# Mictronics/pluto-gps-sim

Hardware: AMD Instinct MI355X
Metric: IQ samples/sec (whole node) at 16 channels; bit-exact int16 IQ vs CPU ref (higher is better)
Workload: dtype f64 NCOs (exact), i32 accumulate of packed int16 I/Q

## Files before the change

### pluto-gps-sim_amd/csrc/gpsbb.hip

```cpp
#include <hip/hip_runtime.h>

#include <algorithm>
#include <cctype>
#include <cmath>
#include <cstdio>
#include <cstdlib>
#include <cstring>
#include <new>
#include <condition_variable>
#include <functional>
#include <mutex>
#include <thread>
#include <chrono>
#include <vector>

#include "gpsbb.h"
#include "gpsbb_kernels.hip.h"
#include "gpsbb_noise.hip.h"
#include "gpsbb_interf.hip.h"
#include "gpsbb_level.hip.h"
#include "gpsbb_events.hip.h"
#include "gpsbb_dense.hip.h"
#include "gpsbb_despread.hip.h"
#include "gpsbb_walk.hip.h"
// ... 9 lines not shown
#ifdef GPSBB_EXPERIMENTS
#define GPSBB_KNOB_LONG(name, dflt) ([](long d) -> long { static const char *const e = getenv(name); return e ? atol(e) : d; }((long)(dflt)))
#define GPSBB_KNOB_SET(name) ([]() -> bool { static const bool v = getenv(name) != nullptr; return v; }())
#else
#define GPSBB_KNOB_LONG(name, dflt) ((long)(dflt))
#define GPSBB_KNOB_SET(name) (false)
#endif


namespace {

constexpr uint64_t kSinCosFnv1a = 0x1c99a5cf84551314ull;

bool make_sincos(int32_t sin512[512], int32_t cos512[512])
{
    const double two_pi = 6.283185307179586476925286766559;
    for (int i = 0; i < 512; i++) {
        const double a = two_pi * (double)i / 512.0;
        sin512[i] = (int32_t)(511.0 * std::sin(a) + 1.0);
        cos512[i] = (int32_t)(511.0 * std::cos(a) + 1.0);
    }
    uint64_t h = 0xcbf29ce484222325ull;
    auto eat = [&h](const int32_t *t) {
        for (int i = 0; i < 512; i++)
            for (int k = 0; k < 4; k++) {
                h ^= (uint8_t)((uint32_t)t[i] >> (8 * k));
                h *= 0x100000001b3ull;
            }
    };
    eat(sin512);
    eat(cos512);
    return h == kSinCosFnv1a;
}

const uint8_t kG2Taps[32][2] = {
    {2, 6}, {3, 7}, {4, 8}, {5, 9}, {1, 9}, {2, 10}, {1, 8}, {2, 9}, {3, 10}, {2, 3}, {3, 4},
    {5, 6}, {6, 7}, {7, 8}, {8, 9}, {9, 10}, {1, 4}, {2, 5}, {3, 6}, {4, 7}, {5, 8}, {6, 9},
    {1, 3}, {4, 6}, {5, 7}, {6, 8}, {7, 9}, {8, 10}, {1, 6}, {2, 7}, {3, 8}, {4, 9}};

void make_ca(int prn, uint8_t ca[GPSBB_CA_LEN])
{
    uint32_t g1 = 0x3ff, g2 = 0x3ff;
    const int t1 = kG2Taps[prn - 1][0], t2 = kG2Taps[prn - 1][1];
    for (int i = 0; i < GPSBB_CA_LEN; i++) {
        const uint32_t o1 = (g1 >> 9) & 1u;
        const uint32_t o2 = ((g2 >> (t1 - 1)) ^ (g2 >> (t2 - 1))) & 1u;
        ca[i] = (uint8_t)(o1 ^ o2);
        const uint32_t f1 = ((g1 >> 2) ^ (g1 >> 9)) & 1u;
        const uint32_t f2 = ((g2 >> 1) ^ (g2 >> 2) ^ (g2 >> 5) ^ (g2 >> 7) ^ (g2 >> 8) ^ (g2 >> 9)) & 1u;
        g1 = ((g1 << 1) | f1) & 0x3ff;
        g2 = ((g2 << 1) | f2) & 0x3ff;
    }
}

bool chan_ok(const gpsbb_chan_t &c, double delt, bool fixed = false)
{
    if (c.prn == 0)
        return true;
    if (c.prn < 0 || c.prn > 32)
        return false;
    if (!std::isfinite(c.f_carr) || !std::isfinite(c.f_code) || !std::isfinite(c.carr_phase) ||
        !std::isfinite(c.code_phase) || !std::isfinite(c.gain))
        return false;
    if (!fixed && (std::signbit(c.carr_phase) || c.carr_phase > 1.0))
        return false;
    if (fixed && (std::signbit(c.carr_phase) || c.carr_phase >= 4294967296.0 || c.carr_phase != std::floor(c.carr_phase)))
        return false;
    if (std::signbit(c.code_phase) || !(c.code_phase < 1023.0))
        return false;
    const double sc = c.f_code * delt, sk = c.f_carr * delt;
    if (!(sc > 0.0 && sc <= 1.5) || !(std::fabs(sk) <= 0.125))
        return false;
    if (!(std::fabs(c.gain) < 2097152.0))
        return false;
    if (c.iword < 0 || c.iword > 59 || c.ibit < 0 || c.ibit > 29 || c.icode < 0 || c.icode > 19)
        return false;
    for (int k = 0; k < GPSBB_N_DWRD; k++)
        if (c.dwrd[k] >> 30)
            return false;
    return true;
}

uint64_t row_bound(double s_abs, double range, int top_e, int nsamp)
{
    if (!(s_abs > 0.0))
        return 4;
    int es;
    std::frexp(s_abs, &es);
    es -= 1;
    const double laps = std::floor((double)nsamp * s_abs / range) + 2.0;
    int binades = top_e - es + 3;
    if (binades < 3)
        binades = 3;
    const double per_lap = 2.0 * binades + 6.0;
    return (uint64_t)(laps * per_lap) + 16;
}

struct CarrDrift {
    int e_lo = 0, n = 0;
    double sa = 0.0, R1 = 0.0;
    bool neg = false;
    double dens[64], cum[65];
    explicit CarrDrift(double s)
    {
        sa = std::fabs(s);
        neg = s < 0.0;
        if (!(sa >= 0x1p-60) || !(sa < 0.25))
            return;
        int es;
        std::frexp(sa, &es);
        es -= 1;
        e_lo = es - 1 < -1 ? es - 1 : -1;
        cum[0] = 0.0;
        for (int e = e_lo; e <= -1; e++) {
            const double ulp = std::ldexp(1.0, e - 52);
            const double q = s / ulp;
            const double delta = (std::nearbyint(q) - q) * ulp;
            dens[n] = delta / sa;
            cum[n + 1] = cum[n] + dens[n] * std::ldexp(1.0, e);
            n++;
        }
        R1 = cum[n];
    }
    double R(double x) const
    {
        if (n == 0 || !(x > std::ldexp(1.0, e_lo)))
            return 0.0;
        if (x >= 1.0)
            return R1;
        const int e = std::ilogb(x);
        const int k = e - e_lo;
        return cum[k] + dens[k] * (x - std::ldexp(1.0, e));
    }
    double advance(double x0, int nsteps, double s) const
    {
        const double u = x0 + (double)nsteps * s;
        const double fl = std::floor(u), end = u - fl;
        const double drift = neg ? -fl * R1 + R(x0) - R(end) : fl * R1 + R(end) - R(x0);
        double v = end + drift;
        v -= std::floor(v);
        return v;
    }
};

double ev_bias_on_grid(double w)
{
#ifdef GPSBB_W_OFF_GRID
    return w;
#else
    return w < 0.25 ? std::ceil(w * 4294967296.0) * 0x1p-32 : w;
#endif
}

bool ev_plan(const gpsbb_chan_t *ch, int nblocks, int nch, double delt, std::vector<EvConst> &out, bool fixed = false)
{
    const size_t nbc = (size_t)nblocks * nch;
    out.resize(nbc);
    const double reach = (double)SPT - 0.5;
    for (int blk = 0; blk < nblocks; blk++) {
        double amp_sum = 0.0;
        for (int i = 0; i < nch; i++) {
            const gpsbb_chan_t &c = ch[(size_t)blk * nch + i];
            EvConst &K = out[(size_t)blk * nch + i];
            memset(&K, 0, sizeof K);
            if (c.prn <= 0)
                continue;
            amp_sum += 512.0 * std::fabs(c.gain) + 1.0;
            const volatile double sc = c.f_code * delt, sk = c.f_carr * delt;
            double S = sk * 512.0;
            if (fixed) {
                const volatile double scaled = 512.0 * 65536.0 * c.f_carr * delt;
                S = (double)(int)std::round(scaled) * 0x1p-16;
            }
            const double aS = std::fabs(S);
            const bool dense_code = !(sc * reach < 1.0);
            if (!(sc >= 0x1p-20) || !(1023.0 + 1040.0 * sc + 2.0 <= (double)EV_CHIP_LEN))
                return false;
            K.S = aS;
            K.sc = sc;
            K.rsc = 1.0 / sc;
            K.down = S < 0.0;
            const double wC = EV_MODEL_ERR * K.rsc + EV_T_EPS;
            double wK = 0.0;
            if (aS == 0.0) {
                K.rS = 0x1p+1000;
                K.kc = 1;
            } else if (aS < 8.0 * EV_MODEL_ERR) {
                K.rS = 0x1p+1000;
                K.kc = -1;
            } else {
                K.rS = 1.0 / aS;
                wK = EV_MODEL_ERR * K.rS + EV_T_EPS;
                const double kc = std::floor((reach + wK) * aS) + 1.0;
                K.kc = kc > (double)EV_KC_MAX ? EV_KC_DENSE : (int)kc;
            }
            K.W = std::max(std::max(wK, wC), EV_T_EPS);
            K.W = ev_bias_on_grid(K.W);
            K.danger = K.W >= 0.25 ? 0x80000000u : (uint32_t)std::ceil(2.0 * K.W * 4294967296.0) + 1u;
            {
                const long floor_ = GPSBB_KNOB_LONG("GPSBB_EV_DANGER", 0);
                if (floor_ > 0 && (uint32_t)floor_ > K.danger)
                    K.danger = (uint32_t)floor_;
            }
            K.tK0 = K.rS * (1.0 + K.W) + 0x1p+20 + K.W;
            K.tC0 = K.rsc * (1.0 + K.W) + 0x1p+20 + K.W;
            K.pd_S8 = aS * 8.0;
            K.pd_dy = aS * 512.0;
            K.pd_sc2 = sc * 2.0;
            K.pd_dx = sc * 128.0;
            if (dense_code && K.kc > 0)
                K.kc = EV_KC_DENSE;
            if (fixed) {
                if (dense_code) {
                    if (!(aS < 64.0))
                        return false;
                    K.kc = EV_KC_DENSE;
                } else {
                    const double kc = std::floor(reach * aS) + 1.0;
                    if (kc > (double)EV_KC_MAX)
                        return false;
                    K.kc = (int)kc;
                    K.rS = aS > 0.0 ? 1.0 / aS : 0x1p+1000;
                    K.W = ev_bias_on_grid(std::max(wC, EV_T_EPS));
                    K.danger = K.W >= 0.25 ? 0x80000000u : (uint32_t)std::ceil(2.0 * K.W * 4294967296.0) + 1u;
                    K.tK0 = K.rS * (1.0 - 0x1p-17) + 0x1p+20;
                    K.tC0 = K.rsc * (1.0 + K.W) + 0x1p+20 + K.W;
                }
            }
            K.danger_le = K.kc < 0 ? 0xffffffffu : K.danger - 1u;
            K.chip_at = (uint32_t)(offsetof(EvLdsLean, chip2) + (size_t)i * sizeof(uint16_t) * EvLdsLean::CHIPS) - (EV_GUARD_HI << 1);
            K.amp_at = (uint32_t)(offsetof(EvLdsLean, amp) + (size_t)i * sizeof(uint32_t) * EvLdsLean::AMP) - (EV_GUARD_HI << 2);
        }
        if (!(amp_sum < 32768.0))
            return false;
    }
    return true;
}

bool lap_eligible(const gpsbb_chan_t *ch, size_t nbc, double delt, bool fixed)
{
    for (size_t k = 0; k < nbc; k++) {
        const gpsbb_chan_t &c = ch[k];
        if (c.prn <= 0)
            continue;
        const volatile double sc = c.f_code * delt, sk = c.f_carr * delt;
        if (!(sc >= 0x1p-20))
            return false;
        if (!fixed && !(std::fabs(sk) >= 0x1p-50) && sk != 0.0)
            return false;
    }
    return true;
}

constexpr int LAP_UNIT_CARR = 4, LAP_UNIT_CODE = 2;
constexpr int LAP_BURST_SHARE = 4;
int lap_unit(int kind, size_t nbc)
{
    long u = kind == NCO_CARR ? GPSBB_KNOB_LONG("GPSBB_LAP_UNIT_CARR", LAP_UNIT_CARR) : GPSBB_KNOB_LONG("GPSBB_LAP_UNIT_CODE", LAP_UNIT_CODE);
    if (nbc <= 256)
        u = 1;
    else if (nbc <= 1024)
        u = kind == NCO_CARR ? std::min(u, 2L) : 1L;
    if (kind == NCO_CODE && u == 0)
        return 0;
    return u < 1 ? 1 : (u > 64 ? 64 : (int)u);
}

void lap_bound(const gpsbb_chan_t *ch, int nblocks, int nch, double delt, int nsamp, bool fixed, uint32_t chunk0[2][GPSBB_MAX_CHAN + 1],
               bool carr_only = false)
{
    for (int kind = 0; kind < 2; kind++) {
        chunk0[kind][0] = kind == 0 ? 0u : chunk0[0][GPSBB_MAX_CHAN];
        for (int i = 0; i < nch; i++) {
            double laps = 0.0;
            for (int blk = 0; blk < nblocks; blk++) {
                const gpsbb_chan_t &c = ch[(size_t)blk * nch + i];
                if (c.prn <= 0 || (kind == NCO_CARR && fixed) || (kind == NCO_CODE && carr_only))
                    continue;
                const double s = kind == NCO_CARR ? std::fabs(c.f_carr * delt) : c.f_code * delt * (1.0 / 1023.0);
                laps += std::floor((std::floor((double)nsamp * s * (1.0 + 0x1p-30)) + 1.0) / (double)std::max(1, lap_unit(kind, (size_t)nblocks * nch))) + 3.0;
            }
            const uint32_t chunks = (uint32_t)((laps + (double)(LAP_WG - 1)) / (double)LAP_WG) + 1u;
            chunk0[kind][i + 1] = chunk0[kind][i] + chunks;
        }
        for (int i = nch; i < GPSBB_MAX_CHAN; i++)
            chunk0[kind][i + 1] = chunk0[kind][i];
    }
}

}


struct WorkPool {
    std::vector<std::thread> th;
    std::mutex m;
    std::condition_variable cv_work, cv_done;
    std::function<void(size_t)> job;
    size_t njobs = 0, next = 0, running = 0;
    unsigned long gen = 0;
    bool stop = false;

    explicit WorkPool(size_t nworkers)
    {
        for (size_t t = 0; t < nworkers; t++)
            th.emplace_back([this] { loop(); });
    }
    ~WorkPool()
    {
        {
            std::lock_guard<std::mutex> g(m);
            stop = true;
        }
        cv_work.notify_all();
        for (auto &t : th)
            t.join();
    }
    void loop()
    {
        unsigned long seen = 0;
        std::unique_lock<std::mutex> lk(m);
        for (;;) {
            cv_work.wait(lk, [&] { return stop || gen != seen; });
            if (stop)
                return;
            seen = gen;
            drain(lk);
        }
    }
    void drain(std::unique_lock<std::mutex> &lk)
    {
        running++;
        while (next < njobs) {
            const size_t j = next++;
            lk.unlock();
            job(j);
            lk.lock();
        }
        if (--running == 0)
            cv_done.notify_all();
    }
    void run(size_t n, std::function<void(size_t)> f)
    {
        std::unique_lock<std::mutex> lk(m);
        job = std::move(f);
        njobs = n;
        next = 0;
        gen++;
// ... 391 lines not shown
        (void)hipFree(h->d_pack);
    if (h->d_noise_tab)
        (void)hipFree(h->d_noise_tab);
    if (h->d_nclip)
        (void)hipFree(h->d_nclip);
    if (h->d_digest.p)
        (void)hipFree(h->d_digest.p);
    if (h->d_level)
        (void)hipFree(h->d_level);
    delete h->pool;
    h->pool = nullptr;
    for_each_stream(h, [](hipStream_t st) { (void)hipStreamDestroy(st); });
    delete h;
}

static hipError_t create_seed_stream(hipStream_t *st);

#ifdef GPSBB_EXPERIMENTS
__global__ void k_park(unsigned long long ticks)
{
    const unsigned long long t0 = wall_clock64();
    while (wall_clock64() - t0 < ticks)
        __builtin_amdgcn_s_sleep(64);
}
#endif

static hipError_t zero_now(gpsbb *h, void *ptr, size_t bytes)
{
#ifdef GPSBB_EXPERIMENTS
    {
        const long park = GPSBB_KNOB_LONG("GPSBB_X_PARK_NULL_MS", 0);
        if (park > 0)
            hipLaunchKernelGGL(k_park, dim3(1), dim3(1), 0, nullptr, (unsigned long long)park * 100000ull);
        if (GPSBB_KNOB_SET("GPSBB_X_NULL_MEMSET"))
            return hipMemsetAsync(ptr, 0, bytes, nullptr);
    }
#endif
    const hipError_t e = hipMemsetAsync(ptr, 0, bytes, h->s_seed);
    return e != hipSuccess ? e : hipStreamSynchronize(h->s_seed);
}

typedef void (*EvKernelFn)(BatchDev, int16_t *);
static EvKernelFn ev_kernel(int g, bool digest);

extern "C" int gpsbb_create(gpsbb_t **out, int device)
{
    if (!out)
        return GPSBB_E_BADARG;
    *out = nullptr;
    int ndev = 0;
    if (hipGetDeviceCount(&ndev) != hipSuccess || ndev <= 0 || device < 0 || device >= ndev)
        return GPSBB_E_NODEVICE;

    int32_t tabs[1024];
    if (!make_sincos(tabs + 512, tabs))
        return GPSBB_E_INTERNAL;
    std::vector<uint32_t> ca(33 * 32, 0u);
    for (int prn = 1; prn <= 32; prn++) {
        uint8_t chips[GPSBB_CA_LEN];
        make_ca(prn, chips);
        for (int i = 0; i < GPSBB_CA_LEN; i++)
            if (chips[i])
                ca[prn * 32 + (i >> 5)] |= 1u << (i & 31);
    }

    gpsbb *h = new (std::nothrow) gpsbb;
    if (!h)
        return GPSBB_E_NOMEM;
    h->device = device;
    auto fail = [&](hipError_t e) {
        h->last_hip = (int)e;
        gpsbb_destroy(h);
        return e == hipErrorOutOfMemory ? GPSBB_E_NOMEM : GPSBB_E_HIP;
    };
    hipError_t e;
    if ((e = hipSetDevice(device)) != hipSuccess) return fail(e);
    hipDeviceProp_t prop;
    if ((e = hipGetDeviceProperties(&prop, device)) != hipSuccess) return fail(e);
    h->sm_count = prop.multiProcessorCount;
    if ((e = create_seed_stream(&h->s_seed)) != hipSuccess) return fail(e);
    {
        const long sp = GPSBB_KNOB_LONG("GPSBB_SYNTH_STREAM_PRIO", 0);
        if (sp != 0) {
            if ((e = hipStreamCreateWithPriority(&h->s_compute, hipStreamNonBlocking, (int)sp)) != hipSuccess) return fail(e);
        } else {
            if ((e = hipStreamCreateWithFlags(&h->s_compute, hipStreamNonBlocking)) != hipSuccess) return fail(e);
        }
    }
    if ((e = create_seed_stream(&h->s_more[0])) != hipSuccess) return fail(e);
    if ((e = hipMalloc((void **)&h->d_tabs, sizeof tabs)) != hipSuccess) return fail(e);
    if ((e = hipMalloc((void **)&h->d_ca, ca.size() * 4)) != hipSuccess) return fail(e);
    if ((e = hipMalloc((void **)&h->d_status, 4)) != hipSuccess) return fail(e);
    if ((e = hipMalloc((void **)&h->d_hz, 64)) != hipSuccess) return fail(e);
    if ((e = hipMalloc((void **)&h->d_clip, 8)) != hipSuccess) return fail(e);
    if ((e = hipMemcpy(h->d_tabs, tabs, sizeof tabs, hipMemcpyHostToDevice)) != hipSuccess) return fail(e);
    if ((e = hipMemcpy(h->d_ca, ca.data(), ca.size() * 4, hipMemcpyHostToDevice)) != hipSuccess) return fail(e);
    if ((e = hipStreamSynchronize(nullptr)) != hipSuccess) return fail(e);
    h->h_ca = ca;
    if ((e = zero_now(h, h->d_status, 4)) != hipSuccess) return fail(e);
    if ((e = zero_now(h, h->d_hz, 64)) != hipSuccess) return fail(e);
    if ((e = zero_now(h, h->d_clip, 8)) != hipSuccess) return fail(e);
    if ((e = hipFuncSetAttribute(reinterpret_cast<const void *>(k_synth), hipFuncAttributeMaxDynamicSharedMemorySize,
                                 (int)sizeof(SynthLds))) != hipSuccess) return fail(e);
    for (int g = 0; g <= EV_STATE_LOG2_MAX; g++) {
        if ((e = hipFuncSetAttribute(reinterpret_cast<const void *>(ev_kernel(g, false)), hipFuncAttributeMaxDynamicSharedMemorySize,
                                     (int)sizeof(EvLdsLean) + EV_PICK_LDS)) != hipSuccess) return fail(e);
        if ((e = hipFuncSetAttribute(reinterpret_cast<const void *>(ev_kernel(g, true)), hipFuncAttributeMaxDynamicSharedMemorySize,
                                     (int)sizeof(EvLdsLean) + EV_PICK_LDS)) != hipSuccess) return fail(e);
    }
    if ((e = hipFuncSetAttribute(reinterpret_cast<const void *>(k_synth_ev_dense), hipFuncAttributeMaxDynamicSharedMemorySize,
                                 (int)sizeof(EvLds) + EV_PICK_LDS)) != hipSuccess) return fail(e);
    if ((e = hipFuncSetAttribute(reinterpret_cast<const void *>(k_synth_ev_fixed), hipFuncAttributeMaxDynamicSharedMemorySize,
                                 (int)sizeof(EvLdsLean) + EV_PICK_LDS)) != hipSuccess) return fail(e);
    if ((e = hipFuncSetAttribute(reinterpret_cast<const void *>(k_synth_pd<true>), hipFuncAttributeMaxDynamicSharedMemorySize,
                                 (int)sizeof(PdLds<true>) + EV_PICK_LDS)) != hipSuccess) return fail(e);
    if ((e = hipFuncSetAttribute(reinterpret_cast<const void *>(k_synth_pd<false>), hipFuncAttributeMaxDynamicSharedMemorySize,
                                 (int)sizeof(PdLds<false>) + EV_PICK_LDS)) != hipSuccess) return fail(e);
    if ((e = hipFuncSetAttribute(reinterpret_cast<const void *>(k_synth_pd<true, true>), hipFuncAttributeMaxDynamicSharedMemorySize,
                                 (int)sizeof(PdLds<true>) + EV_PICK_LDS)) != hipSuccess) return fail(e);
    if ((e = hipFuncSetAttribute(reinterpret_cast<const void *>(k_synth_pd<false, true>), hipFuncAttributeMaxDynamicSharedMemorySize,
                                 (int)sizeof(PdLds<false>) + EV_PICK_LDS)) != hipSuccess) return fail(e);
    *out = h;
    return GPSBB_OK;
}

struct ChainCarry {
    int prn[GPSBB_MAX_CHAN];
    double phase[GPSBB_MAX_CHAN];
};
static void chain_carrier_host(const gpsbb_chan_t *ch, int nblocks, int nch, double delt, int nsamp, double *seed,
                               int nthreads, ChainCarry *carry);

static bool host_seeding_wanted(const gpsbb_batch *b);

typedef void (*LapKernelFn)(BatchDev, LapDev);
static LapKernelFn lap_pass2_kernel(int kind, bool wide, int g)
{
#define GPSBB_P2(W) {{k_lap_pass2<NCO_CODE, W, 0>, k_lap_pass2<NCO_CODE, W, 1>, k_lap_pass2<NCO_CODE, W, 2>}, \
                     {k_lap_pass2<NCO_CARR, W, 0>, k_lap_pass2<NCO_CARR, W, 1>, k_lap_pass2<NCO_CARR, W, 2>}, \
                     {k_lap_pass2_2<W, 0>, k_lap_pass2_2<W, 1>, k_lap_pass2_2<W, 2>}}
    static const LapKernelFn k[2][3][EV_STATE_LOG2_MAX + 1] = {GPSBB_P2(false), GPSBB_P2(true)};
#undef GPSBB_P2
    static_assert(NCO_CODE == 0 && NCO_CARR == 1, "lap_pass2_kernel's table");
    return k[wide ? 1 : 0][kind < 0 ? 2 : kind][g];
}

static EvKernelFn ev_kernel(int g, bool digest)
{
    static const EvKernelFn k[2][EV_STATE_LOG2_MAX + 1] = {{k_synth_ev<0>, k_synth_ev<1>, k_synth_ev<2>},
                                                            {k_synth_ev_digest<0>, k_synth_ev_digest<1>, k_synth_ev_digest<2>}};
    return k[digest ? 1 : 0][g];
}

static int ev_state_log2(const gpsbb_batch *b, bool fixed)
{
    if (!b->ev || !b->laps || b->ev_dense || fixed)
        return 0;
    long g = GPSBB_KNOB_LONG("GPSBB_EV_STATE_LOG2", GPSBB_EV_STATE_LOG2);
    g = g < 0 ? 0 : (g > EV_STATE_LOG2_MAX ? EV_STATE_LOG2_MAX : g);
    while (g > 0 && !ev_granule_fits((int)g))
        g--;
    const size_t nbc = (size_t)b->nblocks * b->nch;
    for (size_t k = 0; k < nbc && g > 0; k++)
        if (!(b->h_evc[k].sc * (double)((TILE << g) + SPT) < (double)(GPSBB_CA_LEN - 1)))
            return 0;
    return (int)g;
}

struct PushTrace {
    double limit_ms = -1.0;
    int n = 0;
    const char *what[32];
    std::chrono::steady_clock::time_point t[32];
    PushTrace()
    {
#ifdef GPSBB_EXPERIMENTS
        const char *e = getenv("GPSBB_PUSH_TRACE");
        if (e)
            limit_ms = atof(e);
#endif
    }
    void start() { n = 0; mark("start"); }
    void mark(const char *w)
    {
        if (limit_ms < 0.0 || n >= 32)
            return;
        what[n] = w;
        t[n++] = std::chrono::steady_clock::now();
    }
    void end()
    {
        if (limit_ms < 0.0 || n < 2)
            return;
        mark("end");
        const double tot = std::chrono::duration<double, std::milli>(t[n - 1] - t[0]).count();
        if (tot < limit_ms)
            return;
        fprintf(stderr, "[gpsbb push %.3f ms]", tot);
        for (int i = 1; i < n; i++)
            fprintf(stderr, " %s %.3f", what[i], std::chrono::duration<double, std::milli>(t[i] - t[i - 1]).count());
        fprintf(stderr, "\n");
    }
};
static thread_local PushTrace g_push_trace;
#define PUSH_MARK(w) g_push_trace.mark(w)

static hipError_t stage_upload(gpsbb_batch *b, void *dst, const void *src, size_t bytes, hipStream_t stream)
{
    const size_t at = (b->stage_used + 63) & ~(size_t)63;
    if (at + bytes > b->stage_cap)
        return hipMemcpyAsync(dst, src, bytes, hipMemcpyHostToDevice, stream);
    memcpy(b->stage + at, src, bytes);
    b->stage_used = at + bytes;
    return hipMemcpyAsync(dst, b->stage + at, bytes, hipMemcpyHostToDevice, stream);
}


static int batch_setup(gpsbb_batch *b, const gpsbb_chan_t *ch, int nblocks, int nch, double delt,
                       int nsamp, unsigned flags, hipStream_t upload_stream)
{
    gpsbb *h = b->h;
    if (!ch || nblocks < 1 || nblocks > 65535 || nch < 1 || nch > GPSBB_MAX_CHAN || nsamp < 1 ||
        !(delt > 0.0) || !std::isfinite(delt) || (flags & ~(GPSBB_CHAIN_CARRIER | GPSBB_FIXED_CARRIER)))
        return GPSBB_E_BADARG;
    const size_t nbc = (size_t)nblocks * nch;
    const bool fixed = (flags & GPSBB_FIXED_CARRIER) != 0;
    for (size_t k = 0; k < nbc; k++)
        if (!chan_ok(ch[k], delt, fixed))
            return GPSBB_E_BADCHAN;

    {
        const size_t need = nbc * (sizeof(gpsbb_chan_t) + sizeof(EvConst) + 8 + 2 * 4 + 5 * 4 +
                                   (size_t)CHAIN_SEG_MAX * (sizeof(ChainDesc) + 8 + 8 + 2 * 4)) + 64 * 1024;
        if (b->upload_done)
            HIPCHK(h, hipEventSynchronize(b->upload_done));
        PUSH_MARK("arena");
        if (need > b->stage_cap) {
            if (b->stage)
                (void)hipHostFree(b->stage);
            b->stage = nullptr;
            b->stage_cap = 0;
            HIPCHK(h, hipHostMalloc((void **)&b->stage, need + need / 4, hipHostMallocDefault));
            b->stage_cap = need + need / 4;
        }
        b->stage_used = 0;
    }
    b->nblocks = nblocks;
    b->nch = nch;
    b->nsamp = nsamp;
    b->delt = delt;
    b->flags = flags;
    b->ntiles = (nsamp + TILE - 1) / TILE;
    if (2ull * nbc * ((unsigned long long)b->ntiles + 1) >= (1ull << 32))
        return GPSBB_E_NOMEM;

    b->ev = h->opt_synth_kernel != 1 && ev_plan(ch, nblocks, nch, delt, b->h_evc, fixed);
    b->ev_dense = false;
    b->ev_all_dense = b->ev;
    if (b->ev)
        for (size_t k = 0; k < nbc; k++) {
            b->ev_dense = b->ev_dense || b->h_evc[k].kc == EV_KC_DENSE;
            b->ev_all_dense = b->ev_all_dense && (ch[k].prn <= 0 || b->h_evc[k].kc == EV_KC_DENSE);
        }
    b->ev_all_dense = b->ev_all_dense && b->ev_dense;
    if (fixed && b->ev_dense && !b->ev_all_dense) {
        b->ev = false;
        b->ev_dense = b->ev_all_dense = false;
    }
    PUSH_MARK("ev_plan");

    const bool lap_ok = b->ev && h->opt_seed_where != 1 && h->opt_seed_where != 2 && h->opt_chain_where != 2 && h->opt_chain_where != 3 &&
                        !GPSBB_KNOB_SET("GPSBB_NO_LAPS") && lap_eligible(ch, nbc, delt, fixed);
    b->host_seed = !lap_ok && !b->d_carry && host_seeding_wanted(b);
    b->laps = lap_ok;
    b->st_log2 = ev_state_log2(b, fixed);
    b->nstates = (b->ntiles + (1 << b->st_log2) - 1) >> b->st_log2;
    const bool chained = !fixed && (flags & GPSBB_CHAIN_CARRIER) && (nblocks > 1 || b->d_carry);
    b->chain_dev = chained && h->opt_chain_where != 1 && !b->host_seed;
    b->chain_fix_seq = h->opt_chain_where == 2;
    b->chain_starts = b->chain_dev && !b->ev;
    b->chain_model = false;
    b->chain_indep = false;
    b->nseg = 1;
    const bool indep_ok = !chained && !b->d_carry && b->ev && !fixed && !b->host_seed && h->opt_chain_where == 0 &&
                          b->ntiles >= (int)GPSBB_KNOB_LONG("GPSBB_INDEP_MIN_TILES", CHAIN_INDEP_MIN_TILES);
    if (!b->laps && ((b->chain_dev && !b->chain_starts) || indep_ok)) {
        double rows_max = 0.0;
        for (size_t k = 0; k < nbc; k++)
            if (ch[k].prn > 0) {
                const double sa = std::fabs(ch[k].f_carr * delt);
                const double r = sa > 0.0 ? ((double)nsamp * sa + 1.0) * (2.0 - std::log2(sa)) : 1.0;
                rows_max = r > rows_max ? r : rows_max;
            }
        int n = (int)(rows_max / (double)GPSBB_KNOB_LONG("GPSBB_SEG_ROWS", CHAIN_SEG_ROWS) + 0.5);
        const int n_cap = b->ntiles / CHAIN_SEG_MIN_TILES;
        n = n > CHAIN_SEG_MAX ? CHAIN_SEG_MAX : n;
        n = n > n_cap ? n_cap : n;
        n = n < 1 ? 1 : n;
        if (b->chain_dev) {
            b->nseg = n;
        } else if (n > 1 && (long)nblocks * n <= CHAIN_MODEL_MAX_SEGS) {
            b->chain_dev = true;
            b->chain_indep = true;
            b->nseg = n;
        }
    }
    b->seg_tiles = (b->ntiles + b->nseg - 1) / b->nseg;
    b->nseg = (b->ntiles + b->seg_tiles - 1) / b->seg_tiles;
    b->chain_model = !b->laps && b->chain_dev && !b->chain_starts && !b->d_carry && h->opt_chain_where != 3 &&
                     (long)nblocks * b->nseg <= CHAIN_MODEL_MAX_SEGS;
    const size_t nvbc = nbc * (size_t)b->nseg;

    b->row_off.assign(nbc + nvbc + 1, 0);
    uint64_t off = 0;
    for (size_t k = 0; k < nbc && !b->laps; k++) {
        b->row_off[k] = off;
        if (ch[k].prn > 0) {
            off += row_bound(ch[k].f_code * delt, 1023.0, 9, nsamp) + 1;
            if (b->ev)
                off += (uint64_t)nsamp / (uint64_t)WALK_ROW_MAX + 1;
        } else {
            off += 1;
        }
    }
    if (!b->laps) {
        const int full = b->seg_tiles * TILE, last = nsamp - (b->nseg - 1) * full;
        const int ns_full = b->nseg == 1 ? nsamp : full, ns_last = b->nseg == 1 ? nsamp : last;
        for (int blk = 0; blk < nblocks; blk++)
            for (int sgi = 0; sgi < b->nseg; sgi++) {
                uint64_t *ro = &b->row_off[nbc + ((size_t)blk * b->nseg + sgi) * nch];
                const int ns = sgi == b->nseg - 1 ? ns_last : ns_full;
                for (int i = 0; i < nch; i++) {
                    const gpsbb_chan_t &c = ch[(size_t)blk * nch + i];
                    ro[i] = 0;
                    if (c.prn > 0 && !fixed) {
                        if (sgi == 0 || sgi == b->nseg - 1)
                            ro[i] = row_bound(std::fabs(c.f_carr * delt), 1.0, -1, ns) + 1 + (b->ev ? (uint64_t)ns / (uint64_t)WALK_ROW_MAX + 1 : 0);
                        else
                            ro[i] = b->row_off[nbc + ((size_t)blk * b->nseg) * nch + i];
                    } else {
                        ro[i] = 1;
                    }
                }
            }
        for (size_t kv = 0; kv < nvbc; kv++) {
            const uint64_t cnt = b->row_off[nbc + kv];
            b->row_off[nbc + kv] = off;
            off += cnt;
        }
    }
    b->row_off[nbc + nvbc] = off;
    b->total_rows = off;

    HIPCHK(h, (hipError_t)b->d_ch.reserve(nbc));
    HIPCHK(h, (hipError_t)b->d_row_off.reserve(nbc + nvbc + 1));
    HIPCHK(h, (hipError_t)b->d_tile_ctr.reserve((size_t)NSETS * ((size_t)nblocks + 1)));
    b->nsets = (int)GPSBB_KNOB_LONG("GPSBB_NSETS", b->chain_dev ? 4 : 3);
    b->nsets = b->nsets < 2 ? 2 : (b->nsets > NSETS ? NSETS : b->nsets);
    b->nsets = b->nsets > b->max_sets ? b->max_sets : b->nsets;
    for (int set = 0; set < b->nsets; set++) {
        HIPCHK(h, (hipError_t)b->d_end[set].reserve(nbc));
        if (b->ev) {
            HIPCHK(h, (hipError_t)b->d_tile_x[set].reserve(2 * nbc * (size_t)b->nstates));
            HIPCHK(h, (hipError_t)b->d_tile_nav[set].reserve(nbc * (size_t)b->nstates));
            HIPCHK(h, (hipError_t)b->d_rows[set].reserve(b->total_rows + 4, b->max_sets == 1 ? (size_t)(b->total_rows / 2) : 0));
            HIPCHK(h, (hipError_t)b->d_row_cnt[set].reserve(nbc + nvbc));
        } else {
            HIPCHK(h, (hipError_t)b->d_rows[set].reserve(b->total_rows + 4));
            HIPCHK(h, (hipError_t)b->d_tile_row[set].reserve(2 * nbc * ((size_t)b->ntiles + 1)));
            HIPCHK(h, (hipError_t)b->d_row_cnt[set].reserve(2 * nbc));
        }
    }
    if (b->ev) {
        HIPCHK(h, (hipError_t)b->d_evc.reserve(nbc));
        HIPCHK(h, stage_upload(b, b->d_evc.p, b->h_evc.data(), nbc * sizeof(EvConst), upload_stream));
    }
    if (fixed) {
        b->h_kph0.assign(nbc, 0u);
        b->h_kstep.assign(nbc, 0);
        for (int i = 0; i < nch; i++) {
            int prev_prn = b->fixed_prev_prn ? b->fixed_prev_prn[i] : 0;
            uint32_t prev_ph = b->fixed_prev_phase ? b->fixed_prev_phase[i] : 0u;
            for (int blk = 0; blk < nblocks; blk++) {
                const gpsbb_chan_t &c = ch[(size_t)blk * nch + i];
                const size_t k = (size_t)blk * nch + i;
                if (c.prn <= 0) {
                    prev_prn = 0;
                    continue;
                }
                const volatile double scaled = 512.0 * 65536.0 * c.f_carr * delt;
                b->h_kstep[k] = (int)std::round(scaled);
                const bool cont = (flags & GPSBB_CHAIN_CARRIER) && c.prn == prev_prn;
                b->h_kph0[k] = cont ? prev_ph : (uint32_t)c.carr_phase;
                prev_ph = b->h_kph0[k] + (uint32_t)nsamp * (uint32_t)b->h_kstep[k];
                prev_prn = c.prn;
            }
        }
        HIPCHK(h, (hipError_t)b->d_kph0.reserve(nbc));
        HIPCHK(h, (hipError_t)b->d_kstep.reserve(nbc));
        HIPCHK(h, stage_upload(b, b->d_kph0.p, b->h_kph0.data(), nbc * 4, upload_stream));
        HIPCHK(h, stage_upload(b, b->d_kstep.p, b->h_kstep.data(), nbc * 4, upload_stream));
    }
    b->h_ch.assign(ch, ch + nbc);
    b->cont0_mask = 0;
    if (b->laps) {
        lap_bound(ch, nblocks, nch, delt, nsamp, fixed, b->lap_chunk0);
        const size_t chunks = (size_t)b->lap_chunk0[1][nch];
        for (int set = 0; set < b->nsets; set++) {
            HIPCHK(h, (hipError_t)b->d_lap_bc[set].reserve(2 * nbc));
            HIPCHK(h, (hipError_t)b->d_lap_lane0[set].reserve(2 * (size_t)nch * ((size_t)nblocks + 1)));
            HIPCHK(h, (hipError_t)b->d_lap_cnt[set].reserve(4 * GPSBB_MAX_CHAN));
            HIPCHK(h, (hipError_t)b->d_lap_rec[set].reserve(chunks * LAP_WG, b->max_sets == 1 ? chunks * LAP_WG / 4 : 0));
            HIPCHK(h, (hipError_t)b->d_lap_agg[set].reserve(chunks, b->max_sets == 1 ? chunks / 4 : 0));
            HIPCHK(h, (hipError_t)b->d_lap_chunk_m[set].reserve(chunks, b->max_sets == 1 ? chunks / 4 : 0));
            HIPCHK(h, (hipError_t)b->d_lap_chunk_bad[set].reserve(chunks, b->max_sets == 1 ? chunks / 4 : 0));
        }
        if (b->chain_dev && b->d_carry && b->carry_prn)
            for (int i = 0; i < nch; i++)
                if (ch[i].prn > 0 && ch[i].prn == b->carry_prn[i])
                    b->cont0_mask |= 1u << i;
    }
    if (b->chain_dev && !b->laps) {
        b->h_cd.resize(nvbc);
        b->h_start0.resize(nvbc);
        for (int i = 0; i < nch; i++) {
            double x = b->d_carry && b->carry_phase ? b->carry_phase[i] : 0.0;
            int prev_prn = b->d_carry && b->carry_prn ? b->carry_prn[i] : 0;
            for (int blk = 0; blk < nblocks; blk++) {
// ... 2955 lines not shown
};
}

extern "C" int gpsbb_test_build_rows(int kind, double x0, double s, unsigned nav0, int nsamp,
                                     gpsbb_test_row_t *rows, int cap, double *x_end, unsigned *nav_end)
{
    HostSink sink{rows, cap, 0, 0};
    uint32_t nav = nav0;
    double x = kind == NCO_CODE ? build_rows<NCO_CODE>(x0, s, nav, nsamp, sink)
                                : build_rows<NCO_CARR>(x0, s, nav, nsamp, sink);
    if (x_end)
        *x_end = x;
    if (nav_end)
        *nav_end = nav;
    return sink.cnt;
}

namespace {
struct HostSinkF64 {
    gpsbb_test_row_t *rows;
    int cap, cnt;
    void row(int32_t n0, uint32_t nav, double x, double S, bool after_wrap)
    {
        if (cnt < cap) {
            rows[cnt].n0 = n0;
            rows[cnt].nav = nav | (after_wrap ? 0x40000000u : 0u);
            rows[cnt].xb = f64_bits(x);
            rows[cnt].inc = (int64_t)f64_bits(S);
        }
        cnt++;
    }
    void nav_fetch(uint32_t) {}
    void table_index_512() {}
};
}

extern "C" int gpsbb_test_build_rows_f64(int kind, double x0, double s, unsigned nav0, int nsamp,
                                         gpsbb_test_row_t *rows, int cap, double *x_end, unsigned *nav_end)
{
    HostSinkF64 sink{rows, cap, 0};
    uint32_t nav = nav0;
    double x = kind == NCO_CODE ? build_rows_f64<NCO_CODE>(x0, s, nav, nsamp, sink)
                                : build_rows_f64<NCO_CARR>(x0, s, nav, nsamp, sink);
    if (x_end)
        *x_end = x;
    if (nav_end)
        *nav_end = nav;
    return sink.cnt;
}

extern "C" double gpsbb_test_carr_predict(double x0, double s, int n)
{
    const CarrDrift d(s);
    return d.advance(x0, n, s);
}

extern "C" double gpsbb_test_fixed_tile_index(uint32_t ph0, int32_t step, int t)
{
    return fixed_tile_index(ph0, step, t);
}

extern "C" int gpsbb_test_model_err(gpsbb_batch_t *b, double *maxima, unsigned long long *counts, int *which)
{
    if (!b || !maxima || !counts)
        return GPSBB_E_BADARG;
    gpsbb *h = b->h;
    if (!b->ran || !b->ev)
        return GPSBB_E_STATE;
    const int rc = gpsbb_sync(h);
    if (rc != GPSBB_OK)
        return rc;
    const BatchDev p = batch_dev(b, b->last_set);
    double *d_mx = nullptr;
    unsigned long long *d_cnt = nullptr;
    const size_t mx_bytes = sizeof(double) * GPSBB_MAX_CHAN * ME_NQ, cnt_bytes = sizeof(unsigned long long) * GPSBB_MAX_CHAN * MEC_NQ;
    HIPCHK(h, hipMalloc((void **)&d_mx, mx_bytes));
    HIPCHK(h, hipMalloc((void **)&d_cnt, cnt_bytes));
    HIPCHK(h, hipMemsetAsync(d_mx, 0, mx_bytes, h->s_compute));
    HIPCHK(h, hipMemsetAsync(d_cnt, 0, cnt_bytes, h->s_compute));
    const size_t threads = (size_t)b->nblocks * b->nch * b->ntiles;
    const dim3 grid((unsigned)((threads + 255) / 256));
    if (b->ev_all_dense)
        hipLaunchKernelGGL(k_model_err_pd, grid, dim3(256), 0, h->s_compute, p, d_mx, d_cnt);
    else
        hipLaunchKernelGGL(k_model_err_ev, grid, dim3(256), 0, h->s_compute, p, d_mx, d_cnt);
    HIPCHK(h, hipGetLastError());
    HIPCHK(h, hipStreamSynchronize(h->s_compute));
    HIPCHK(h, hipMemcpy(maxima, d_mx, mx_bytes, hipMemcpyDeviceToHost));
    HIPCHK(h, hipMemcpy(counts, d_cnt, cnt_bytes, hipMemcpyDeviceToHost));
    (void)hipFree(d_mx);
    (void)hipFree(d_cnt);
    if (which)
        *which = b->ev_all_dense ? 2 : 1;
    return GPSBB_OK;
}

extern "C" int gpsbb_test_state_log2(gpsbb_batch_t *b)
{
    return b ? b->st_log2 : GPSBB_E_BADARG;
}

extern "C" int gpsbb_test_table_digest(gpsbb_batch_t *b, unsigned long long out[3])
{
    if (!b || !out || !b->ran || !b->ev)
        return GPSBB_E_STATE;
    gpsbb *h = b->h;
    const int rc = gpsbb_sync(h);
    if (rc != GPSBB_OK)
        return rc;
    const BatchDev p = batch_dev(b, b->last_set);
    auto mix = [](unsigned long long z) { z ^= z >> 31; z *= 0xBF58476D1CE4E5B9ull; z ^= z >> 29; return z; };
    const size_t nst = (size_t)b->nstates;
    const size_t nx = (size_t)b->nblocks * 2 * b->nch * nst, nn = (size_t)b->nblocks * b->nch * nst, ne = (size_t)b->nblocks * b->nch;
    const int dg = b->ev_dense || (b->flags & GPSBB_FIXED_CARRIER) ? 0 : (int)GPSBB_KNOB_LONG("GPSBB_EV_STATE_LOG2", GPSBB_EV_STATE_LOG2);
    const int tstep = 1 << (dg > b->st_log2 ? dg : b->st_log2);
    std::vector<unsigned long long> hx(nx);
    std::vector<uint32_t> hn(nn);
    std::vector<gpsbb_chan_state_t> he(ne);
    HIPCHK(h, hipMemcpy(hx.data(), p.tile_x, nx * 8, hipMemcpyDeviceToHost));
    HIPCHK(h, hipMemcpy(hn.data(), p.tile_nav, nn * 4, hipMemcpyDeviceToHost));
    HIPCHK(h, hipMemcpy(he.data(), p.end, ne * sizeof(gpsbb_chan_state_t), hipMemcpyDeviceToHost));
    out[0] = out[1] = out[2] = 0;
    std::vector<gpsbb_chan_t> hc(ne);
    HIPCHK(h, hipMemcpy(hc.data(), p.ch, ne * sizeof(gpsbb_chan_t), hipMemcpyDeviceToHost));
    for (size_t k = 0; k < ne; k++) {
        if (hc[k].prn <= 0)
            continue;
        const size_t blk = k / (size_t)b->nch, i = k % (size_t)b->nch;
        for (int kind = 0; kind < 2; kind++)
            for (int t = 0; t < b->ntiles; t += tstep) {
                const size_t at = (blk * 2 * b->nch + 2 * i + kind) * (size_t)b->ntiles + t;
                out[0] += mix(hx[(blk * 2 * b->nch + 2 * i + kind) * nst + (t >> b->st_log2)] + 0x9E3779B97F4A7C15ull * (at + 1));
            }
        for (int t = 0; t < b->ntiles; t += tstep) {
            const size_t at = k * (size_t)b->ntiles + t;
            out[1] += mix((unsigned long long)(hn[k * nst + (t >> b->st_log2)] & 3u) + 0x9E3779B97F4A7C15ull * (at + 1));
        }
        unsigned long long w[5];
        memcpy(w, &he[k], sizeof w);
        for (int q = 0; q < 4; q++)
            out[2] += mix(w[q] + 0x9E3779B97F4A7C15ull * (k * 5 + q + 1));
        out[2] += mix((unsigned long long)(uint32_t)he[k].codeCA + 0x9E3779B97F4A7C15ull * (k * 5 + 5));
    }
    return GPSBB_OK;
}

extern "C" void gpsbb_test_budgets(double out[3])
{
    out[0] = EV_MODEL_ERR * 0x1p+32;
    out[1] = EV_T_EPS * 0x1p+32;
    out[2] = (double)PD_BAND;
}

extern "C" unsigned long long gpsbb_test_row_bound(int kind, double s_abs, int nsamp)
{
    return kind == NCO_CODE ? row_bound(s_abs, 1023.0, 9, nsamp) : row_bound(s_abs, 1.0, -1, nsamp);
}

extern "C" long long gpsbb_test_read_pattern(gpsbb_t *h, const void *d_src, size_t bytes)
{
    if (!h || !d_src)
        return GPSBB_E_BADARG;
    const int rows = 32, cols = 2442;
    const size_t per_wave = (size_t)rows * cols * 8;
    size_t waves = bytes / per_wave;
    waves -= waves % 4;
    if (waves < 4)
        return GPSBB_E_BADARG;
    double *d_sink = nullptr;
    if (hipMalloc((void **)&d_sink, 8) != hipSuccess)
        return GPSBB_E_NOMEM;
    hipLaunchKernelGGL(k_read_pattern, dim3((unsigned)(waves / 4)), dim3(256), 0, h->s_compute, (const double *)d_src, rows, cols, d_sink);
    const hipError_t e = hipStreamSynchronize(h->s_compute);
    (void)hipFree(d_sink);
    return e == hipSuccess ? (long long)(waves * per_wave) : (long long)GPSBB_E_HIP;
}

extern "C" unsigned long long gpsbb_test_despread_exact(gpsbb_batch *b) { return b ? b->ds_last_exact : 0ull; }
extern "C" float gpsbb_test_despread_ms(gpsbb_batch *b)
{
    float ms = -1.0f;
    if (!b || !b->ds_ev[0] || !b->ds_ev[1] || hipEventElapsedTime(&ms, b->ds_ev[0], b->ds_ev[1]) != hipSuccess)
        return -1.0f;
    return ms;
}

#ifdef GPSBB_WG_TRACE
namespace {
unsigned long long *g_trace_buf = nullptr;
unsigned g_trace_cap = 0;
}
extern "C" int gpsbb_test_wg_trace_begin(unsigned cap)
{
    if (hipDeviceSynchronize() != hipSuccess)
        return GPSBB_E_HIP;
    if (cap > g_trace_cap) {
        if (g_trace_buf)
            (void)hipFree(g_trace_buf);
        g_trace_buf = nullptr;
        g_trace_cap = 0;
        if (hipMalloc((void **)&g_trace_buf, (size_t)cap * WG_TRACE_WORDS * 8) != hipSuccess)
            return GPSBB_E_NOMEM;
        g_trace_cap = cap;
    }
    const unsigned zero = 0;
    if (hipMemcpyToSymbol(HIP_SYMBOL(g_wg_trace), &g_trace_buf, sizeof g_trace_buf) != hipSuccess ||
        hipMemcpyToSymbol(HIP_SYMBOL(g_wg_trace_cap), &cap, sizeof cap) != hipSuccess ||
        hipMemcpyToSymbol(HIP_SYMBOL(g_wg_trace_n), &zero, sizeof zero) != hipSuccess)
        return GPSBB_E_HIP;
    return hipDeviceSynchronize() == hipSuccess ? GPSBB_OK : GPSBB_E_HIP;
}
extern "C" long gpsbb_test_wg_trace_read(unsigned long long *out, unsigned cap)
{
    if (hipDeviceSynchronize() != hipSuccess)
        return GPSBB_E_HIP;
    unsigned n = 0;
    if (hipMemcpyFromSymbol(&n, HIP_SYMBOL(g_wg_trace_n), sizeof n) != hipSuccess)
        return GPSBB_E_HIP;
    const unsigned have = n < g_trace_cap ? n : g_trace_cap, take = have < cap ? have : cap;
    if (take && hipMemcpy(out, g_trace_buf, (size_t)take * WG_TRACE_WORDS * 8, hipMemcpyDeviceToHost) != hipSuccess)
        return GPSBB_E_HIP;
    return (long)n;
}
#endif
#endif
```

### pluto-gps-sim_amd/csrc/gpsbb_events.hip.h

```cpp
#ifndef GPSBB_EVENTS_HIP_H
#define GPSBB_EVENTS_HIP_H

#include <cstddef>
#include <type_traits>

#include "gpsbb_kernels.hip.h"

namespace gpsbb_impl {

#ifndef GPSBB_EV_WG
#define GPSBB_EV_WG 1024
#endif
constexpr int EV_WG = GPSBB_EV_WG;
constexpr int EV_WAVES = EV_WG / 64;
constexpr int EV_KC_MAX = 4;
constexpr int EV_AMP_PAD = EV_KC_MAX;
constexpr int EV_AMP_STRIDE = 512 + EV_AMP_PAD + 4;
constexpr int EV_CHIP_LEN = 1024 + 544;
constexpr int EV_KC_DENSE = EV_KC_MAX + 1;
#ifndef GPSBB_EV_CHUNK
#define GPSBB_EV_CHUNK 4
#endif
constexpr int EV_CHUNK = GPSBB_EV_CHUNK;
constexpr int PD_CHUNK = 2;
constexpr int EV_ROW_DISCARD = 15;

#ifndef EV_MODEL_ERR
#define EV_MODEL_ERR 0x1p-30
#define GPSBB_EV_MODEL_ERR_OWN 1
#endif
#ifndef EV_T_EPS
#define EV_T_EPS 0x1p-29
#endif
#define EV_GUARD 0x1p+20

#ifndef GPSBB_EV_STATE_LOG2
#define GPSBB_EV_STATE_LOG2 1
#endif
constexpr int EV_STATE_LOG2_MAX = 2;
static_assert(GPSBB_EV_STATE_LOG2 >= 0 && GPSBB_EV_STATE_LOG2 <= EV_STATE_LOG2_MAX, "state granule: 1, 2 or 4 tiles");
constexpr bool ev_granule_fits(int g) { return ((double)(TILE << g) + (double)(SPT - 1)) * 0x1p-44 + 1.5 * 0x1p-32 <= EV_MODEL_ERR; }
#ifdef GPSBB_EV_MODEL_ERR_OWN
static_assert(ev_granule_fits(EV_STATE_LOG2_MAX), "the model of the largest state granule must stay inside the error budget");
#endif

#define GPSBB_EV_SETTLE_CLAIM() asm volatile("s_waitcnt vmcnt(0)" ::: "memory")

constexpr int EV_CHIP_LEN_SHORT = 1104;
constexpr int EV_AMP_STRIDE_LONG = 512 + 272 + EV_AMP_PAD;
template <int AMP_STRIDE, int CHIP_LEN>
struct EvLdsT {
    static constexpr int AMP = AMP_STRIDE, CHIPS = CHIP_LEN;
    static constexpr bool UNMASKED = AMP_STRIDE >= EV_AMP_STRIDE_LONG;
    uint32_t amp[GPSBB_MAX_CHAN][AMP_STRIDE];
    uint32_t D[EV_WAVES][16][64];
    double tstate[EV_WAVES][2][2 * GPSBB_MAX_CHAN];
    uint16_t chip2[GPSBB_MAX_CHAN][CHIP_LEN];
};
typedef EvLdsT<EV_AMP_STRIDE, EV_CHIP_LEN> EvLds;
typedef EvLdsT<EV_AMP_STRIDE_LONG, EV_CHIP_LEN_SHORT> EvLdsLean;
static_assert(sizeof(EvLds) <= 160 * 1024 && sizeof(EvLdsLean) <= 160 * 1024, "one workgroup per CU: 160 KB of LDS");
static_assert(offsetof(EvLdsLean, D) < 65536 && offsetof(EvLds, D) < 65536, "the difference arrays are addressed with a 16-bit offset");

__device__ __forceinline__ uint32_t lds_addr_of(const void *p)
{
    return (uint32_t)(uintptr_t)(__attribute__((address_space(3))) const void *)p;
}
template <class T>
__device__ __forceinline__ T lds_read_at(uint32_t a)
{
    return *(__attribute__((address_space(3))) const T *)(uintptr_t)a;
}


typedef uint32_t ev_u32x4 __attribute__((ext_vector_type(4)));

template <class T>
__device__ __forceinline__ void lds_write_at(uint32_t a, T v)
{
    *(__attribute__((address_space(3))) T *)(uintptr_t)a = v;
}

constexpr uint32_t EV_SAT_HI_C = 0x4130000fu;
#define EV_SAT_HI EV_SAT_HI_C

template <class LDS>
__device__ __forceinline__ void ev_d_add(uint32_t &drow, int wave, uint32_t pos_hi, uint32_t v)
{
    asm volatile("v_add_u32_sdwa %0, %1, %2 dst_sel:BYTE_1 dst_unused:UNUSED_PRESERVE src0_sel:DWORD src1_sel:BYTE_0\n\t"
                 "ds_add_u32 %0, %3 offset:%4"
                 : "+v"(drow)
                 : "s"(wave << 4), "v"(pos_hi), "v"(v), "n"(offsetof(LDS, D))
                 );
}

__device__ __forceinline__ uint32_t signed_by(uint32_t x, uint32_t m) { return (x ^ m) - m; }

template <class T>
__device__ __forceinline__ T scalar_load(const T *p)
{
    typedef const __attribute__((address_space(4))) T *cptr_t;
    return *(cptr_t)(uintptr_t)p;
}

template <bool FIXED, class LDS>
__device__ __forceinline__ uint32_t ev_exact_run_body(LDS &L, int wave, int lane, int i, const EvConst *kbi, const double *tile_x,
                                                      int ntiles, uint32_t nb, int n_off, uint32_t fx_phase, int32_t fx_step)
{
    constexpr bool fixed = FIXED;
    const bool down = kbi->down != 0;
    const double S = down ? -kbi->S : kbi->S, sc = kbi->sc;
    const double xt = tile_x[(size_t)(2 * i) * ntiles], yt = tile_x[(size_t)(2 * i + 1) * ntiles];
    int64_t wraps = 0;
    double x = code_jump(xt, sc, (int64_t)n_off, &wraps);
    uint32_t dbm = (wraps > 0 ? (nb >> 1) & 1u : nb & 1u) ? 0xffffffffu : 0u;
    const uint32_t dbm_next = ((nb >> 1) & 1u) ? 0xffffffffu : 0u;
    const double s = S * (1.0 / 512.0);
    double cp = carr_jump(yt * (1.0 / 512.0), s, (int64_t)n_off);
    uint32_t prev = 0, first = 0;
    uint32_t ph = fx_phase + (uint32_t)n_off * (uint32_t)fx_step;
#pragma unroll 1
    for (int j = 0; j < SPT; j++) {
        const int it = fixed ? (int)((ph >> 16) & 0x1ffu)
                             : ((int)(cp * 512.0) & 511);
        const int ci = (int)x;
        const uint32_t m = (uint32_t)(int32_t)(int8_t)(L.chip2[i][ci] & 0xffu) ^ dbm;
        const uint32_t v = signed_by(L.amp[i][down ? 511 - it : it], m);
        if (j == 0)
            first = v;
        else
            __hip_atomic_fetch_add(&L.D[wave][j - 1][lane], v - prev, __ATOMIC_RELAXED, __HIP_MEMORY_SCOPE_WORKGROUP);
        prev = v;
        if (code_step(x, sc))
            dbm = dbm_next;
        carr_step(cp, s);
        ph += (uint32_t)fx_step;
    }
    return first;
}

struct EvFixed {
    const uint32_t *ph;
    const int32_t *st;
    int n0;
};

template <class LDS>
__device__ __noinline__ uint32_t ev_exact_run(LDS &L, int wave, int lane, int i, const EvConst *kbi, const double *tile_x,
                                              int ntiles, uint32_t nb, int n_off)
{
    return ev_exact_run_body<false>(L, wave, lane, i, kbi, tile_x, ntiles, nb, n_off, 0u, 0);
}
template <class LDS>
__device__ __noinline__ uint32_t ev_exact_run_fixed(LDS &L, int wave, int lane, int i, const EvConst *kbi, const double *tile_x,
                                                    int ntiles, uint32_t nb, int n_off, uint32_t fx_phase, int32_t fx_step)
{
    return ev_exact_run_body<true>(L, wave, lane, i, kbi, tile_x, ntiles, nb, n_off, fx_phase, fx_step);
}

struct EvK {
    double S, rS, sc, rsc;
    uint32_t danger;
    uint32_t chip_base;
    uint32_t amp_base;
};
constexpr uint32_t EV_GUARD_HI = 0x41300000u;
template <class LDS>
__device__ __forceinline__ EvK ev_load_k(const LDS &L, const EvConst *kb, int i)
{
    EvK k;
    typedef uint32_t u32x8 __attribute__((ext_vector_type(8)));
    typedef uint32_t u32x4 __attribute__((ext_vector_type(4)));
    const char *ki = reinterpret_cast<const char *>(kb) + ((uint32_t)i << 7);
    const u32x8 a = scalar_load(reinterpret_cast<const u32x8 *>(ki));
    const u32x4 c = scalar_load(reinterpret_cast<const u32x4 *>(ki + offsetof(EvConst, danger_le)));
    k.S = __hiloint2double((int)a[1], (int)a[0]);
    k.rS = __hiloint2double((int)a[3], (int)a[2]);
    k.sc = __hiloint2double((int)a[5], (int)a[4]);
    k.rsc = __hiloint2double((int)a[7], (int)a[6]);
    k.danger = c[0];
    if (LDS::UNMASKED) {
        k.chip_base = c[1];
        k.amp_base = c[2];
    } else {
        k.chip_base = lds_addr_of(&L.chip2[i][0]) - (EV_GUARD_HI << 1);
        k.amp_base = lds_addr_of(&L.amp[i][0]) - (EV_GUARD_HI << 2);
    }
    return k;
}

template <int KC>
struct EvHalf {
    uint32_t hk[KC];
    uint32_t hc;
    int c0;
    unsigned long long um;
// ... 575 lines not shown
```

### pluto-gps-sim_amd/csrc/gpsbb_testhooks.h

```cpp
#ifndef GPSBB_TESTHOOKS_H
#define GPSBB_TESTHOOKS_H
#include <stdint.h>
#ifdef __cplusplus
extern "C" {
#endif

typedef struct gpsbb_test_row {
    int32_t n0;
    uint32_t nav;
    uint64_t xb;
    int64_t inc;
} gpsbb_test_row_t;

double gpsbb_test_carr_jump(double x, double s, long long n);
double gpsbb_test_code_jump(double x, double s, long long n, long long *wraps);
int gpsbb_test_build_rows(int kind, double x0, double s, unsigned nav0, int nsamp, gpsbb_test_row_t *rows,
                          int cap, double *x_end, unsigned *nav_end);
int gpsbb_test_build_rows_f64(int kind, double x0, double s, unsigned nav0, int nsamp, gpsbb_test_row_t *rows,
                              int cap, double *x_end, unsigned *nav_end);
unsigned long long gpsbb_test_row_bound(int kind, double s_abs, int nsamp);
double gpsbb_test_carr_predict(double x0, double s, int n);
double gpsbb_test_fixed_tile_index(unsigned ph0, int step, int t);

#define GPSBB_TEST_ME_NQ 11
#define GPSBB_TEST_MEC_NQ 4
struct gpsbb_batch;
int gpsbb_test_model_err(struct gpsbb_batch *b, double *maxima, unsigned long long *counts, int *which);
unsigned long long gpsbb_test_despread_exact(struct gpsbb_batch *b);
float gpsbb_test_despread_ms(struct gpsbb_batch *b);
void gpsbb_test_budgets(double out[3]);

#ifdef __cplusplus
}
#endif
#endif
```

Before: 610.3 billion.

## Default event state granule to four tiles with a per-granule error budget

Raises the default event-synthesis state granule from two tiles to four. Because the larger granule's model error no longer fits the old budget, the error budget now depends on the granule, and the plan's guard window W is derived from that budget. Planning is reordered so the lap eligibility and granule are chosen before ev_plan runs, with fallbacks that replan if the widened budget would change kernel selection or the final granule. Fewer stored states should reduce per-tile state work and traffic, at the cost of wider guard windows that may trigger more exact-fallback checks.

New measurement: 634.4 billion, median of 6. +4.0%, better.

```diff
diff --git a/pluto-gps-sim_amd/csrc/gpsbb.hip b/pluto-gps-sim_amd/csrc/gpsbb.hip
--- a/pluto-gps-sim_amd/csrc/gpsbb.hip
+++ b/pluto-gps-sim_amd/csrc/gpsbb.hip
@@ -185,7 +185,14 @@
 #endif
 }
 
-bool ev_plan(const gpsbb_chan_t *ch, int nblocks, int nch, double delt, std::vector<EvConst> &out, bool fixed = false)
+inline bool ev_dense_code(const gpsbb_chan_t &c, double delt)
+{
+    const volatile double sc = c.f_code * delt;
+    return !(sc * ((double)SPT - 0.5) < 1.0);
+}
+
+bool ev_plan(const gpsbb_chan_t *ch, int nblocks, int nch, double delt, std::vector<EvConst> &out, bool fixed = false,
+             double model_err = EV_MODEL_ERR, bool *same_kernels = nullptr)
 {
     const size_t nbc = (size_t)nblocks * nch;
     out.resize(nbc);
@@ -206,14 +213,14 @@
                 S = (double)(int)std::round(scaled) * 0x1p-16;
             }
             const double aS = std::fabs(S);
-            const bool dense_code = !(sc * reach < 1.0);
+            const bool dense_code = ev_dense_code(c, delt);
             if (!(sc >= 0x1p-20) || !(1023.0 + 1040.0 * sc + 2.0 <= (double)EV_CHIP_LEN))
                 return false;
             K.S = aS;
             K.sc = sc;
             K.rsc = 1.0 / sc;
             K.down = S < 0.0;
-            const double wC = EV_MODEL_ERR * K.rsc + EV_T_EPS;
+            const double wC = model_err * K.rsc + EV_T_EPS;
             double wK = 0.0;
             if (aS == 0.0) {
                 K.rS = 0x1p+1000;
@@ -223,9 +230,12 @@
                 K.kc = -1;
             } else {
                 K.rS = 1.0 / aS;
-                wK = EV_MODEL_ERR * K.rS + EV_T_EPS;
+                wK = model_err * K.rS + EV_T_EPS;
                 const double kc = std::floor((reach + wK) * aS) + 1.0;
                 K.kc = kc > (double)EV_KC_MAX ? EV_KC_DENSE : (int)kc;
+                if (same_kernels && K.kc == EV_KC_DENSE && model_err != (double)(EV_MODEL_ERR) &&
+                    !(std::floor((reach + (EV_MODEL_ERR * K.rS + EV_T_EPS)) * aS) + 1.0 > (double)EV_KC_MAX))
+                    *same_kernels = false;
             }
             K.W = std::max(std::max(wK, wC), EV_T_EPS);
             K.W = ev_bias_on_grid(K.W);
@@ -923,14 +933,20 @@
     return k[digest ? 1 : 0][g];
 }
 
-static int ev_state_log2(const gpsbb_batch *b, bool fixed)
-{
-    if (!b->ev || !b->laps || b->ev_dense || fixed)
-        return 0;
+static int ev_state_log2_wanted()
+{
     long g = GPSBB_KNOB_LONG("GPSBB_EV_STATE_LOG2", GPSBB_EV_STATE_LOG2);
     g = g < 0 ? 0 : (g > EV_STATE_LOG2_MAX ? EV_STATE_LOG2_MAX : g);
     while (g > 0 && !ev_granule_fits((int)g))
         g--;
+    return (int)g;
+}
+
+static int ev_state_log2(const gpsbb_batch *b, bool fixed, int cap)
+{
+    if (!b->ev || !b->laps || b->ev_dense || fixed)
+        return 0;
+    long g = std::min(ev_state_log2_wanted(), cap);
     const size_t nbc = (size_t)b->nblocks * b->nch;
     for (size_t k = 0; k < nbc && g > 0; k++)
         if (!(b->h_evc[k].sc * (double)((TILE << g) + SPT) < (double)(GPSBB_CA_LEN - 1)))
@@ -1025,7 +1041,21 @@
     if (2ull * nbc * ((unsigned long long)b->ntiles + 1) >= (1ull << 32))
         return GPSBB_E_NOMEM;
 
-    b->ev = h->opt_synth_kernel != 1 && ev_plan(ch, nblocks, nch, delt, b->h_evc, fixed);
+    const bool lap_pre = h->opt_seed_where != 1 && h->opt_seed_where != 2 && h->opt_chain_where != 2 && h->opt_chain_where != 3 &&
+                         !GPSBB_KNOB_SET("GPSBB_NO_LAPS") && lap_eligible(ch, nbc, delt, fixed);
+    bool dense_code = false;
+    for (size_t k = 0; k < nbc && !dense_code; k++)
+        dense_code = ch[k].prn > 0 && ev_dense_code(ch[k], delt);
+    int g_plan = fixed || !lap_pre || dense_code ? 0 : ev_state_log2_wanted();
+    double planned_err = ev_model_err(g_plan);
+    bool same_kernels = true;
+    b->ev = h->opt_synth_kernel != 1 && ev_plan(ch, nblocks, nch, delt, b->h_evc, fixed, planned_err, &same_kernels);
+    if (b->ev && !same_kernels) {
+        while (g_plan > 0 && ev_model_err(g_plan) != (double)(EV_MODEL_ERR))
+            g_plan--;
+        planned_err = ev_model_err(g_plan);
+        b->ev = ev_plan(ch, nblocks, nch, delt, b->h_evc, fixed, planned_err);
+    }
     b->ev_dense = false;
     b->ev_all_dense = b->ev;
     if (b->ev)
@@ -1040,11 +1070,14 @@
     }
     PUSH_MARK("ev_plan");
 
-    const bool lap_ok = b->ev && h->opt_seed_where != 1 && h->opt_seed_where != 2 && h->opt_chain_where != 2 && h->opt_chain_where != 3 &&
-                        !GPSBB_KNOB_SET("GPSBB_NO_LAPS") && lap_eligible(ch, nbc, delt, fixed);
+    const bool lap_ok = b->ev && lap_pre;
     b->host_seed = !lap_ok && !b->d_carry && host_seeding_wanted(b);
     b->laps = lap_ok;
-    b->st_log2 = ev_state_log2(b, fixed);
+    b->st_log2 = ev_state_log2(b, fixed, g_plan);
+    if (b->ev && ev_model_err(b->st_log2) != planned_err) {
+        if (!ev_plan(ch, nblocks, nch, delt, b->h_evc, fixed, ev_model_err(b->st_log2)))
+            return GPSBB_E_INTERNAL;
+    }
     b->nstates = (b->ntiles + (1 << b->st_log2) - 1) >> b->st_log2;
     const bool chained = !fixed && (flags & GPSBB_CHAIN_CARRIER) && (nblocks > 1 || b->d_carry);
     b->chain_dev = chained && h->opt_chain_where != 1 && !b->host_seed;
@@ -4306,6 +4339,20 @@
     out[2] = (double)PD_BAND;
 }
 
+extern "C" int gpsbb_test_plan_w(gpsbb_batch_t *b, double *out, int cap)
+{
+    if (!b || !out)
+        return GPSBB_E_BADARG;
+    if (!b->ev)
+        return GPSBB_E_STATE;
+    const size_t nbc = (size_t)b->nblocks * b->nch;
+    if (cap < 0 || (size_t)cap < nbc || b->h_evc.size() != nbc)
+        return GPSBB_E_BADARG;
+    for (size_t k = 0; k < nbc; k++)
+        out[k] = b->h_evc[k].W * 0x1p+32;
+    return (int)nbc;
+}
+
 extern "C" unsigned long long gpsbb_test_row_bound(int kind, double s_abs, int nsamp)
 {
     return kind == NCO_CODE ? row_bound(s_abs, 1023.0, 9, nsamp) : row_bound(s_abs, 1.0, -1, nsamp);
diff --git a/pluto-gps-sim_amd/csrc/gpsbb_events.hip.h b/pluto-gps-sim_amd/csrc/gpsbb_events.hip.h
--- a/pluto-gps-sim_amd/csrc/gpsbb_events.hip.h
+++ b/pluto-gps-sim_amd/csrc/gpsbb_events.hip.h
@@ -35,13 +35,19 @@
 #define EV_GUARD 0x1p+20
 
 #ifndef GPSBB_EV_STATE_LOG2
-#define GPSBB_EV_STATE_LOG2 1
+#define GPSBB_EV_STATE_LOG2 2
 #endif
 constexpr int EV_STATE_LOG2_MAX = 2;
 static_assert(GPSBB_EV_STATE_LOG2 >= 0 && GPSBB_EV_STATE_LOG2 <= EV_STATE_LOG2_MAX, "state granule: 1, 2 or 4 tiles");
-constexpr bool ev_granule_fits(int g) { return ((double)(TILE << g) + (double)(SPT - 1)) * 0x1p-44 + 1.5 * 0x1p-32 <= EV_MODEL_ERR; }
+constexpr double ev_granule_bound(int g) { return ((double)(TILE << g) + (double)(SPT - 1)) * 0x1p-44 + 1.5 * 0x1p-32; }
+constexpr double ev_model_err(int g) { return g <= 1 ? (double)(EV_MODEL_ERR) : 1.25 * (double)(EV_MODEL_ERR); }
+constexpr bool ev_granule_fits(int g) { return ev_granule_bound(g) <= ev_model_err(g); }
 #ifdef GPSBB_EV_MODEL_ERR_OWN
-static_assert(ev_granule_fits(EV_STATE_LOG2_MAX), "the model of the largest state granule must stay inside the error budget");
+constexpr bool ev_budget_is_twice_the_bound(int g) { return 2.0 * ev_granule_bound(g) <= ev_model_err(g) + 0.01 * 0x1p-32; }
+static_assert(ev_granule_fits(0) && ev_granule_fits(1) && ev_granule_fits(EV_STATE_LOG2_MAX) && EV_STATE_LOG2_MAX == 2,
+              "the model of every state granule must stay inside its error budget");
+static_assert(ev_budget_is_twice_the_bound(0) && ev_budget_is_twice_the_bound(1) && ev_budget_is_twice_the_bound(2),
+              "the budget of a state granule is twice its derived bound (to 0.01 units)");
 #endif
 
 #define GPSBB_EV_SETTLE_CLAIM() asm volatile("s_waitcnt vmcnt(0)" ::: "memory")
diff --git a/pluto-gps-sim_amd/csrc/gpsbb_testhooks.h b/pluto-gps-sim_amd/csrc/gpsbb_testhooks.h
--- a/pluto-gps-sim_amd/csrc/gpsbb_testhooks.h
+++ b/pluto-gps-sim_amd/csrc/gpsbb_testhooks.h
@@ -29,6 +29,7 @@
 unsigned long long gpsbb_test_despread_exact(struct gpsbb_batch *b);
 float gpsbb_test_despread_ms(struct gpsbb_batch *b);
 void gpsbb_test_budgets(double out[3]);
+int gpsbb_test_plan_w(struct gpsbb_batch *b, double *out, int cap);
 
 #ifdef __cplusplus
 }
```
